# valeoai/PAFUSE

Hardware: AMD Instinct MI355X
Metric: hypotheses/sec through DDIM loop (H3WB 133-kp, P=20, T=10) (higher is better)
Workload: dtype bf16x3 (every fp32 GEMM operand as the exact sum of three bf16 slices, six bf16 MFMA products per fp32-equivalent product, fp32 accumulate; activations, LayerNorm, softmax, attention and everything in memory fp32; the residual stream stored centred on its row means)

## Files before the change

__graft_entry__.py:

```python
import os
import subprocess
import sys

ROOT = os.path.dirname(os.path.abspath(__file__))
if ROOT not in sys.path:
    sys.path.insert(0, ROOT)

SRC = os.path.join(ROOT, "pafuse_amd", "csrc", "pafuse_hip.hip")
CSRC = os.path.join(ROOT, "pafuse_amd", "csrc")
DEPS = [SRC, os.path.join(ROOT, "include", "pafuse_hip.h")] + [os.path.join(CSRC, f) for f in
                                                              ("kernels.hpp", "hgemm.hpp", "xgemm.hpp", "sgemm.hpp", "train_kernels.hpp", "train_host.inc")]
OUT = os.path.join(ROOT, "pafuse_amd", "libpafuse_hip.so")
from pafuse_amd.build_flags import HIPCC_FLAGS

FLAGS_NOTE = OUT + ".flags"


def _stale(out, deps):
    if (not os.path.exists(out)) or any(os.path.getmtime(d) > os.path.getmtime(out) for d in deps):
        return True
    try:
        with open(FLAGS_NOTE) as f:
            return f.read().strip() != " ".join(HIPCC_FLAGS)
    except OSError:
        return True


def hipcc_compile(args, out):
    hipcc = os.environ.get("HIPCC", "/opt/rocm/bin/hipcc")
    cmd = [hipcc] + HIPCC_FLAGS + list(args) + ["-o", out]
    print("[build]", " ".join(cmd), file=sys.stderr, flush=True)
    r = subprocess.run(cmd, stderr=subprocess.PIPE, text=True)
    noise = "is not a recognized feature for this target"
    sys.stderr.write("".join(l for l in r.stderr.splitlines(True) if noise not in l))
# ... 70 lines not shown
```

include/pafuse_hip.h:

```cpp
#ifndef PAFUSE_HIP_H
#define PAFUSE_HIP_H

#include <stddef.h>
#include <stdint.h>

#ifdef __cplusplus
extern "C" {
#endif

#define PAFUSE_OK 0
#define PAFUSE_E_ARG (-1)
#define PAFUSE_E_SHAPE (-2)
#define PAFUSE_E_WORKSPACE (-3)
#define PAFUSE_E_HIP (-4)
#define PAFUSE_E_RANGE (-5)

#define PAFUSE_MAX_DEPTH 16
#define PAFUSE_MAX_PARTS 4

typedef struct pafuse_block_weights {
    const float *norm1_w, *norm1_b;
    const float *qkv_w, *qkv_b;
    const float *proj_w, *proj_b;
    const float *norm2_w, *norm2_b;
// ... 88 lines not shown
    const float *W;
    const void *Wsplit;
    const float *bias;
    const float *resid;
    float *out_x, *out_n;
    const float *post_w, *post_b;
    float post_eps;
    const float *pos;
    int32_t posJ, posF;
    const float *next_w, *next_b;
    float next_eps;
    const float *head_w, *head_b;
    float *out_head;
    float *ln_stats;
    const void *A_img;
    const void *resid_img;
    void *out_x_img, *out_n_img;
    const float *rowscale;
    int32_t rs_temporal, rs_J, rs_FJ;
    float *out_pre;
} pafuse_rowln_args;
int pafuse_linear_rowln(const pafuse_rowln_args *a, void *stream);
int pafuse_linear_rowln_group(const pafuse_rowln_args *a, int32_t n, int32_t shared_grid, void *stream);

int pafuse_layernorm(const float *x, const float *w, const float *b, float *out, int64_t M, int32_t C, float eps,
                     void *stream);

int pafuse_attention(const float *qkv, float *o, int64_t nseq, int32_t L, int32_t C, int32_t heads, int64_t group,
                     int64_t group_stride, int64_t seq_stride, int64_t tok_stride, void *stream);

int pafuse_attention_backward(const float *qkv, const float *d_o, float *dqkv, int64_t nseq, int32_t L, int32_t C, int32_t heads,
                              int64_t group, int64_t group_stride, int64_t seq_stride, int64_t tok_stride, void *stream);
size_t pafuse_linear_weight_grad_bytes(void);
int pafuse_linear_weight_grad(const float *dY, const float *X, float *dW, float *db, int64_t M, int32_t N, int32_t K,
                              int32_t operand_bf16, void *workspace, size_t workspace_bytes, void *stream);

typedef struct pafuse_lnb_args {
    const float *dy, *x, *w;
    float eps;
    const float *add;
    float *dx;
    const float *drop;
    int32_t temporal, J, FJ;
    float *out_scaled;
    float *dw, *db, *dbranch;
    int64_t M;
// ... 214 lines not shown
```

pafuse_amd/_lib.py:

```python
import ctypes as C
import os

_HERE = os.path.dirname(os.path.abspath(__file__))
LIB_PATH = os.path.join(_HERE, "libpafuse_hip.so")

MAX_DEPTH = 16
MAX_PARTS = 4
f32p = C.POINTER(C.c_float)
i32p = C.POINTER(C.c_int32)


BLOCK_FIELDS = ("norm1_w", "norm1_b", "qkv_w", "qkv_b", "proj_w", "proj_b",
                "norm2_w", "norm2_b", "fc1_w", "fc1_b", "fc2_w", "fc2_b")


class BlockWeights(C.Structure):
    _names = ("norm1_w", "norm1_b", "qkv_w", "qkv_b", "proj_w", "proj_b",
              "norm2_w", "norm2_b", "fc1_w", "fc1_b", "fc2_w", "fc2_b",
              "qkv_ws", "proj_ws", "fc1_ws", "fc2_ws",
              "qkv_ls", "qkv_lt", "fc1_ls", "fc1_lt",
              "qkv_hs", "qkv_hb", "qkv_hl", "fc2_hp")
    _fields_ = [(n, C.c_void_p) for n in _names]


# ... 39 lines not shown
                [(n, C.c_int32) for n in ("operand_bf16", "ln_folded", "h_residual_only")] +
                [(n, C.c_void_p) for n in ("x", "xn", "image", "stats")] + [("row0", C.c_int64), ("nrows", C.c_int64)])


class DDIMStep(C.Structure):
    _fields_ = [("time", C.c_int64), ("last", C.c_int32),
                ("sqrt_recip_acp", C.c_double), ("sqrt_recipm1_acp", C.c_double),
                ("sqrt_alpha_next", C.c_double), ("c", C.c_double), ("sigma", C.c_double)]


SIGNATURES = {
    "pafuse_version": (C.c_char_p, []),
    "pafuse_last_error": (C.c_char_p, []),
    "pafuse_abi_version": (C.c_int, []),
    "pafuse_linear": (C.c_int, [C.c_void_p, C.c_void_p, C.c_void_p, C.c_void_p, C.c_int64, C.c_int32, C.c_int32,
                                C.c_int32, C.c_void_p]),
    "pafuse_split_weights_bytes": (C.c_size_t, [C.c_int64, C.c_int64]),
    "pafuse_split_image_bytes": (C.c_size_t, [C.c_int64, C.c_int64, C.c_int32]),
    "pafuse_split_weights": (C.c_int, [C.c_void_p, C.c_int32, C.c_int32, C.c_int32, C.c_void_p, C.c_void_p]),
    "pafuse_linear_split": (C.c_int, [C.c_void_p, C.c_void_p, C.c_void_p, C.c_void_p, C.c_int64, C.c_int32, C.c_int32,
                                      C.c_int32, C.c_void_p]),
    "pafuse_linear_rowln": (C.c_int, [C.POINTER(RowLNArgs), C.c_void_p]),
    "pafuse_linear_rowln_group": (C.c_int, [C.POINTER(RowLNArgs), C.c_int32, C.c_int32, C.c_void_p]),
    "pafuse_hsplit_rows": (C.c_int, [C.c_void_p, C.c_int64, C.c_int32, C.c_void_p, C.c_void_p]),
    "pafuse_xsplit_rows": (C.c_int, [C.c_void_p, C.c_int64, C.c_int32, C.c_void_p, C.c_void_p]),
    "pafuse_linear_x": (C.c_int, [C.c_void_p, C.c_void_p, C.c_void_p, C.c_void_p, C.c_void_p, C.c_int64, C.c_int32, C.c_int32,
                                  C.c_int32, C.c_void_p]),
    "pafuse_linear_h": (C.c_int, [C.c_void_p, C.c_void_p, C.c_void_p, C.c_void_p, C.c_void_p, C.c_int64, C.c_int32, C.c_int32,
                                  C.c_int32, C.c_void_p]),
    "pafuse_qkv_attention_image": (C.c_int, [C.c_int32, C.c_void_p, C.c_void_p, C.c_void_p, C.c_void_p, C.c_void_p, C.c_int64, C.c_int64,
                                             C.c_int32, C.c_int32, C.c_int32, C.c_int64, C.c_int64, C.c_int64, C.c_int64, C.c_float, C.c_void_p]),
    "pafuse_mlp_h": (C.c_int, [C.c_void_p, C.c_void_p, C.c_void_p, C.c_void_p, C.c_void_p, C.c_void_p, C.c_void_p, C.c_void_p,
                               C.c_int64, C.c_int32, C.c_float, C.c_void_p]),
    "pafuse_layernorm": (C.c_int, [C.c_void_p, C.c_void_p, C.c_void_p, C.c_void_p, C.c_int64, C.c_int32, C.c_float,
                                   C.c_void_p]),
    "pafuse_attention": (C.c_int, [C.c_void_p, C.c_void_p, C.c_int64, C.c_int32, C.c_int32, C.c_int32, C.c_int64,
                                   C.c_int64, C.c_int64, C.c_int64, C.c_void_p]),
    "pafuse_attention_backward": (C.c_int, [C.c_void_p, C.c_void_p, C.c_void_p, C.c_int64, C.c_int32, C.c_int32, C.c_int32,
                                            C.c_int64, C.c_int64, C.c_int64, C.c_int64, C.c_void_p]),
    "pafuse_linear_weight_grad_bytes": (C.c_size_t, []),
    "pafuse_linear_weight_grad": (C.c_int, [C.c_void_p, C.c_void_p, C.c_void_p, C.c_void_p, C.c_int64, C.c_int32, C.c_int32,
                                            C.c_int32, C.c_void_p, C.c_size_t, C.c_void_p]),
    "pafuse_train_unit_bytes": (C.c_size_t, [C.c_int64, C.c_int32, C.c_int32]),
    "pafuse_layernorm_backward": (C.c_int, [C.POINTER(LnbArgs), C.c_void_p, C.c_size_t, C.c_void_p]),
    "pafuse_linear_input_grad": (C.c_int, [C.c_void_p, C.c_void_p, C.c_void_p, C.c_void_p, C.c_int64, C.c_int32, C.c_int32,
                                           C.c_int32, C.c_int32, C.c_void_p, C.c_size_t, C.c_void_p]),
# ... 146 lines not shown
```

pafuse_amd/csrc/kernels.hpp:

```cpp
#pragma once
#include <hip/hip_runtime.h>
#include <stdint.h>

#include <utility>

namespace pafuse {

typedef float f32x16 __attribute__((ext_vector_type(16)));
typedef float f32x4 __attribute__((ext_vector_type(4)));

constexpr int BK = 32;
constexpr int LDK = 36;

typedef __bf16 bf16x8 __attribute__((ext_vector_type(8)));
__device__ __forceinline__ bf16x8 to_bf16x8(const f32x4 lo, const f32x4 hi) {
    bf16x8 v;
#pragma unroll
    for (int i = 0; i < 4; ++i) v[i] = (__bf16)lo[i], v[4 + i] = (__bf16)hi[i];
    return v;
}

#ifdef PAFUSE_MFMA_K8
typedef __bf16 bf16x4_t __attribute__((ext_vector_type(4)));
typedef short s16x4_t __attribute__((ext_vector_type(4)));
// ... 234 lines not shown
    v += __shfl_xor(v, 32);
    return half_wave_sum(v);
}

enum { EPI_BIAS = 0, EPI_ROWLN = 1, EPI_ROWLN_TRAIN = 2 };

enum { MODE_F32 = 0, MODE_BF16 = 1, MODE_BF16X3 = 2, MODE_F16X2 = 3, MODE_BF16X3_IMAGES = 4 };
constexpr bool mode_valid(int m) { return m >= MODE_F32 && m <= MODE_BF16X3_IMAGES; }
constexpr bool mode_split(int m) { return m >= MODE_BF16X3; }
constexpr bool mode_images(int m) { return m >= MODE_F16X2; }
constexpr int image_elem_bytes(int m) { return m == MODE_BF16X3_IMAGES ? 6 : 4; }
enum { WLAYOUT_PLAIN = 0, WLAYOUT_ROWLN = 1, WLAYOUT_M16 = 2 };

struct GemmParams {
    const float* A;
    const float* W;
    const float* bias;
    float* out;
    int64_t M;
    int N, K;
    int mode;
    const uint8_t* Wsplit;
    int wlayout;
    int act;
    float* out_act;
    const float* dact_u;
    const float* resid;
    float* out_x;
    float* out_n;
    const float* post_w;
    const float* post_b;
    float post_eps;
    const float* pos;
    int posJ, posF;
    const float* next_w;
    const float* next_b;
    float next_eps;
    const float* head_w;
    const float* head_b;
    float* out_head;
    float* ln_stats;
    const float* ln_in;
    const float* ln_s;
    const uint8_t* Ah;
    const uint8_t* Wh;
    uint8_t* out_h;
// ... 1061 lines not shown
        constexpr auto need = [](int nth) { return (size_t)VEC + 5 * BN + (size_t)NW * 32 * (32 * nth + 4); };
        constexpr int NTH = (NT % 2 == 0 && need(2) <= RINGF) ? 2 : 1;
        static_assert(need(NTH) <= RINGF, "epilogue scratch must fit the ring");
        epilogue_rows_h<WN, NT, BM, NW, NTH, false, 2>(acc, p, m0, n0, wm, wn, r, h, wave, lane, smem, 1.0f);
    } else {
        epilogue_row_per_lane<WN, NT, BM, EPI, VEC>(acc, p, m0, n0, wm, wn, r, h, smem);
    }
}

template <int WM, int WN, int NT, int EPI, int NSTAGE, int MINW, int ABL = 0, int BKC = 32>
__global__ void __launch_bounds__(WM* WN * 64, MINW) gemm_dma_kernel(const GemmParams p) {
    PAFUSE_XQ_GUARD();
    extern __shared__ __attribute__((aligned(16))) float smem[];
    gemm_dma_tile<WM, WN, NT, EPI, NSTAGE, ABL, BKC>(p, blockIdx.x, gridDim.x, smem);
}

constexpr int GROUP_MAX = 4;
struct GroupedGemmParams {
    GemmParams p[GROUP_MAX];
    int first[GROUP_MAX + 1];
    int n;
};

template <int EPI>
__global__ void __launch_bounds__(256, 2) grouped_rowln_kernel(const GroupedGemmParams g) {
    PAFUSE_XQ_GUARD();
    extern __shared__ __attribute__((aligned(16))) float smem[];
    const int b = blockIdx.x;
    int s = 0;
#pragma unroll
    for (int i = 1; i < GROUP_MAX; ++i)
        if (i < g.n && b >= g.first[i]) s = i;
    const GemmParams& p = g.p[s];
    const int lb = b - g.first[s], nb = g.first[s + 1] - g.first[s];
    switch (p.N) {
        case 384: gemm_dma_tile<2, 2, 6, EPI, 2, 0, 16, false>(p, lb, nb, smem); break;
        case 256: gemm_dma_tile<2, 2, 4, EPI, 2, 0, 16, false>(p, lb, nb, smem); break;
        case 224: gemm_dma_tile<4, 1, 7, EPI, 2, 0, 16, false>(p, lb, nb, smem); break;
        default: break;
    }
}

struct AttnParams {
    const float* qkv;
    float* o;
    uint8_t* o_h;
    int64_t nseq;
    int L, C, heads, d;
    int64_t group, group_stride, seq_stride, tok_stride;
    float scale;
};

template <int ITEMS>
__device__ __forceinline__ void attn_item(int64_t i, int64_t nseq, int heads, int64_t& seq, int& head) {
    if (nseq % 8 == 0 && ((nseq / 8) * heads) % ITEMS == 0) {
        const int64_t blk = i / ITEMS;
        const int lo = (int)(blk % 8);
        const int64_t u = (blk / 8) * ITEMS + (i % ITEMS);
        head = (int)(u % heads);
        seq = (u / heads) * 8 + lo;
    } else {
// ... 2565 lines not shown
```

pafuse_amd/csrc/pafuse_hip.hip:

```cpp
#include "../../include/pafuse_hip.h"

#include <hip/hip_runtime.h>

#include <algorithm>
#include <cmath>
#include <cstdarg>
#include <cstdio>
#include <cstdlib>
#include <cstring>
#include <type_traits>

#include "kernels.hpp"
#include "hgemm.hpp"
#include "xgemm.hpp"
#include "sgemm.hpp"
#include "train_kernels.hpp"

using namespace pafuse;

namespace {

thread_local char g_err[512] = "";

int fail(int code, const char* fmt, ...) {
    va_list ap;
    va_start(ap, fmt);
    vsnprintf(g_err, sizeof g_err, fmt, ap);
    va_end(ap);
    return code;
}

int check_launch(const char* what) {
    hipError_t e = hipGetLastError();
    if (e != hipSuccess) return fail(PAFUSE_E_HIP, "%s: %s", what, hipGetErrorString(e));
    return PAFUSE_OK;
}

inline size_t align_up(size_t x, size_t a = 256) { return (x + a - 1) / a * a; }
// ... 231 lines not shown
        case 8: return launch_strip2<NB, 8>(p, s);
        default: return fail(PAFUSE_E_ARG, "strip GEMM: epilogue options %d", flags);
    }
}
int strip2_bias(const GemmParams& p, hipStream_t s) {
    if (p.N % 128 == 0) return launch_strip2_flags<8>(p, s);
    if (p.N % 112 == 0) return launch_strip2_flags<7>(p, s);
    return launch_strip2_flags<6>(p, s);
}

int wsplit_chunk(int N, bool whole_row) { return (whole_row && (N == 384 || N == 288 || N == 256 || N == 224)) ? 16 : 32; }

template <int WM, int WN, int NT, int EPI, int NSTAGE, int MINW, int BKC = 32>
int launch_gemm_dma(const GemmParams& p, hipStream_t s) {
    using T = DmaTile<WM, WN, NT, BKC>;
    constexpr size_t lds = (size_t)NSTAGE * T::STAGE_BYTES;
    static_assert(lds <= 160 * 1024, "LDS budget");
    static_assert(EPI == EPI_BIAS || (size_t)7 * T::BM * WN * sizeof(float) <= lds, "cross-wave reduction scratch must fit");
    if (!p.Wsplit) return fail(PAFUSE_E_ARG, "split-precision GEMM without a pre-split weight image");
    if (p.K % BKC) return fail(PAFUSE_E_SHAPE, "split GEMM: K=%d is not a multiple of %d", p.K, BKC);
    const int64_t tiles = (p.M + T::BM - 1) / T::BM * (p.N / T::BN);
    if (tiles <= 0 || tiles > 0x7fffffff) return fail(PAFUSE_E_ARG, "gemm grid out of range");
    return launch<gemm_dma_kernel<WM, WN, NT, EPI, NSTAGE, MINW, 0, BKC>>("gemm_dma_kernel", (unsigned)tiles, T::NTHR, lds, s, p);
}

template <int WM, int WN, int NT, int EPI, int NSTAGE, int BKC, int MINW, bool HRES = false>
int launch_hgemm(const GemmParams& p, hipStream_t s) {
    using T = HTile<WM, WN, NT, BKC>;
    constexpr size_t lds = (size_t)NSTAGE * T::STAGE_BYTES;
    static_assert(lds <= 160 * 1024, "LDS budget");
    static_assert(EPI == EPI_BIAS || (size_t)7 * T::BM * WN * sizeof(float) <= lds, "cross-wave reduction scratch must fit");
    if (!p.Ah || !p.Wh) return fail(PAFUSE_E_ARG, "f16x2 GEMM without the H images of its operands");
    if (p.K % BKC || p.K <= 0 || p.N % T::BN) return fail(PAFUSE_E_SHAPE, "f16x2 GEMM: N=%d, K=%d do not fit the %d-column tile", p.N, p.K, T::BN);
    if (HRES && !p.resid_h) return fail(PAFUSE_E_ARG, "f16x2 whole-row GEMM: no H-image residual");
    const int64_t tiles = (p.M + T::BM - 1) / T::BM * (p.N / T::BN);
    if (tiles <= 0 || tiles > 0x7fffffff) return fail(PAFUSE_E_ARG, "gemm grid out of range");
    return launch<hgemm_kernel<WM, WN, NT, EPI, NSTAGE, BKC, MINW, HRES>>("hgemm_kernel", (unsigned)tiles, T::NTHR, lds, s, p);
}

bool hgemm_width(int C) { return C == 384 || C == 256 || C == 224; }
bool hgemm_plain_n(int N) { return N > 0 && (N % 128 == 0 || N % 224 == 0); }

int hgemm_bias(const GemmParams& p, hipStream_t s) {
    if (p.M <= 0) return PAFUSE_OK;
    if (p.N % 128 == 0) return launch_hgemm<4, 2, 2, EPI_BIAS, 3, 16, 2>(p, s);
    if (p.N % 224 == 0) return launch_hgemm<4, 1, 7, EPI_BIAS, 3, 16, 2>(p, s);
// ... 118 lines not shown

template <int EPI>
int gemm_rowln_as(const GemmParams& p0, hipStream_t s) {
    GemmParams p = p0;
    if (p.mode == MODE_BF16X3 && (debug_f32_mask() & 2)) p.mode = MODE_F32;
    if (p.M <= 0) return PAFUSE_OK;
    if (p.K % BK || p.K <= 0) return fail(PAFUSE_E_SHAPE, "rowln: K=%d must be a positive multiple of 32", p.K);
    if (p.mode == MODE_F16X2 || p.mode == MODE_BF16X3_IMAGES) {
        if constexpr (EPI == EPI_ROWLN) return p.mode == MODE_F16X2 ? hgemm_rowln(p, s) : xgemm_rowln(p, s);
        else return fail(PAFUSE_E_ARG, "training has no image-pipeline kernels");
    }
    if constexpr (EPI == EPI_ROWLN_TRAIN) {
        if (p.mode == MODE_BF16X3) {
            switch (p.N) {
                case 384: return launch_gemm_dma<2, 2, 6, EPI, 2, 2, 16>(p, s);
                case 256: return launch_gemm_dma<2, 2, 4, EPI, 2, 2, 16>(p, s);
                case 224: if (p.M >= 4096) return launch_gemm_dma<4, 1, 7, EPI, 2, 2, 16>(p, s); break;
                default: break;
            }
            p.mode = MODE_F32;
        }
    }
    if constexpr (EPI == EPI_ROWLN) {
        if (p.mode == MODE_BF16X3) {
            switch (p.N) {
                case 384: return launch_gemm_dma<2, 2, 6, EPI, 2, 2, 16>(p, s);
                case 256: return launch_gemm_dma<2, 2, 4, EPI, 2, 2, 16>(p, s);
                case 288: return launch_gemm_dma<2, 3, 3, EPI, 2, 2, 16>(p, s);
                case 224:
                    return p.M >= 4096 ? launch_gemm_dma<4, 1, 7, EPI, 2, 2, 16>(p, s) : launch_gemm_dma<2, 1, 7, EPI, 2, 2, 16>(p, s);
                case 128: return launch_gemm<1, 4, 1, EPI, 1, 1, 1, 2>(p, s);
                case 64: return launch_gemm<1, 2, 1, EPI, 1, 1, 1, 2>(p, s);
                default: break;
            }
        } else if (p.mode != MODE_F32) {
            switch (p.N) {
                case 384: return launch_gemm<1, 4, 3, EPI, 1, 1, 1, 1>(p, s);
                case 288: return launch_gemm<1, 3, 3, EPI, 1, 1, 1, 1>(p, s);
                case 256: return launch_gemm<2, 2, 4, EPI, 1, 2, 1, 1>(p, s);
                case 224: return launch_gemm<1, 7, 1, EPI, 1, 1, 1, 1>(p, s);
                case 128: return launch_gemm<1, 4, 1, EPI, 1, 1, 1, 1>(p, s);
                case 64: return launch_gemm<1, 2, 1, EPI, 1, 1, 1, 1>(p, s);
                default: break;
            }
        }
    }
    switch (p.N) {
        case 384: return launch_gemm<1, 4, 3, EPI, 1, 1, 1>(p, s);
        case 288: return launch_gemm<1, 3, 3, EPI, 1, 1, 1>(p, s);
        case 256: return launch_gemm<2, 2, 4, EPI, 1, 2, 1>(p, s);
        case 224: return launch_gemm<1, 7, 1, EPI, 1, 1, 1>(p, s);
        case 128: return launch_gemm<1, 4, 1, EPI, 1, 1, 1>(p, s);
        case 64: return launch_gemm<1, 2, 1, EPI, 1, 1, 1>(p, s);
        default: return fail(PAFUSE_E_SHAPE, "no whole-row kernel for channel width %d (have 64,128,224,256,288,384)", p.N);
    }
}

int gemm_rowln(const GemmParams& p, hipStream_t s) { return gemm_rowln_as<EPI_ROWLN>(p, s); }
int gemm_rowln_train(const GemmParams& p, hipStream_t s) { return gemm_rowln_as<EPI_ROWLN_TRAIN>(p, s); }

bool group_ok_rowln(const GemmParams& p) {
    return p.mode == MODE_BF16X3 && p.Wsplit && (p.N == 384 || p.N == 256 || (p.N == 224 && p.M >= 4096)) && p.K % 16 == 0 && p.K > 0 &&
           !(debug_f32_mask() & 2);
}

template <bool ROWLN>
int gemm_group(const GemmParams* ps, int n, hipStream_t s, bool shared_grids) {
    bool ok = ROWLN && shared_grids && n >= 2 && n <= GROUP_MAX;
    for (int i = 0; i < n && ok; ++i) ok = ps[i].M > 0 && group_ok_rowln(ps[i]);
    if (!ok) {
        for (int i = 0; i < n; ++i) {
            const int rc = ROWLN ? gemm_rowln(ps[i], s) : gemm_bias(ps[i], s);
            if (rc) return rc;
        }
        return PAFUSE_OK;
    }
    int order[GROUP_MAX];
    double cost[GROUP_MAX];
    int64_t tiles[GROUP_MAX];
    for (int i = 0; i < n; ++i) {
        const GemmParams& p = ps[i];
        int bm, bn;
        bm = p.N == 224 ? 128 : 64, bn = p.N;
        tiles[i] = (p.M + bm - 1) / bm * (p.N / bn);
        cost[i] = (double)bm * bn * p.K;
        order[i] = i;
    }
    std::sort(order, order + n, [&](int a, int b) { return cost[a] > cost[b]; });
    GroupedGemmParams g{};
    g.n = n;
    int64_t first = 0;
    for (int k = 0; k < n; ++k) {
        g.p[k] = ps[order[k]];
        g.first[k] = (int)first;
        first += (tiles[order[k]] + 7) / 8 * 8;
        if (first > 0x7fffffff) return fail(PAFUSE_E_ARG, "grouped gemm grid out of range");
    }
    g.first[n] = (int)first;
    for (int k = n + 1; k <= GROUP_MAX; ++k) g.first[k] = (int)first;
    constexpr size_t lds = 2 * DmaTile<2, 2, 6, 16>::STAGE_BYTES;
    static_assert(lds >= 2 * DmaTile<2, 2, 4, 16>::STAGE_BYTES && lds >= 2 * DmaTile<4, 1, 7, 16>::STAGE_BYTES && lds <= 80 * 1024, "LDS");
    return launch<grouped_rowln_kernel<EPI_ROWLN>>("grouped_rowln_kernel", (unsigned)first, 256, lds, s, g);
}

bool width_supported(int C) { return C == 384 || C == 288 || C == 256 || C == 224 || C == 128 || C == 64; }

template <int LP, int DP, int NW>
int launch_attn(const AttnParams& p, hipStream_t s) {
    constexpr int ITEMS = NW / (LP / 16);
    constexpr size_t lds = (size_t)2 * ITEMS * LP * (DP + 4) * sizeof(float);
    const int64_t nitems = p.nseq * p.heads;
    const int64_t grid = (nitems + ITEMS - 1) / ITEMS;
    if (grid > 0x7fffffff) return fail(PAFUSE_E_ARG, "attention grid out of range");
    return launch<attn_kernel<LP, DP, NW>>("attn_kernel", (unsigned)grid, NW * 64, lds, s, p);
}

template <int DP>
int launch_attn_long(const AttnParams& p, hipStream_t s) {
    constexpr size_t lds = (size_t)2 * ATTN_LONG_LP * (DP + 4) * sizeof(float);
    static_assert(lds <= 160 * 1024, "LDS");
    const int64_t grid = p.nseq * p.heads;
    if (grid > 0x7fffffff) return fail(PAFUSE_E_ARG, "attention grid out of range");
    return launch<attn_long_kernel<DP>>("attn_long_kernel", (unsigned)grid, 1024, lds, s, p);
}

// ... 534 lines not shown
    g.A = a->A, g.W = a->W, g.bias = a->bias, g.M = a->M, g.N = a->N, g.K = a->K, g.mode = mode;
    g.Wsplit = mode == MODE_BF16X3 ? (const uint8_t*)a->Wsplit : nullptr;
    g.resid = a->resid, g.out_x = a->out_x, g.out_n = a->out_n;
    g.post_w = a->post_w, g.post_b = a->post_b, g.post_eps = a->post_eps;
    g.pos = a->pos, g.posJ = a->posJ, g.posF = a->posF;
    g.next_w = a->next_w, g.next_b = a->next_b, g.next_eps = a->next_eps;
    g.head_w = a->head_w, g.head_b = a->head_b, g.out_head = a->out_head;
    g.ln_stats = a->ln_stats;
    if (img) {
        g.Ah = (const uint8_t*)a->A_img, g.Wh = (const uint8_t*)a->Wsplit;
        g.resid_h = (const uint8_t*)a->resid_img;
        g.out_xh = (uint8_t*)a->out_x_img, g.out_nh = (uint8_t*)a->out_n_img;
    }
    g.rowscale = a->rowscale, g.rs_temporal = a->rs_temporal, g.rs_J = a->rs_J, g.rs_FJ = a->rs_FJ, g.out_pre = a->out_pre;
    return PAFUSE_OK;
}

int pafuse_linear_rowln(const pafuse_rowln_args* a, void* stream) {
    StreamDevice on_stream_device(stream);
    GemmParams g;
    const int rc = rowln_params(a, g);
    if (rc) return rc;
    if (g.M == 0) return PAFUSE_OK;
    return a->training ? gemm_rowln_train(g, (hipStream_t)stream) : gemm_rowln(g, (hipStream_t)stream);
}

int pafuse_linear_rowln_group(const pafuse_rowln_args* a, int32_t n, int32_t shared_grid, void* stream) {
    StreamDevice on_stream_device(stream);
    if (!a || n < 1 || n > GROUP_MAX) return fail(PAFUSE_E_ARG, "linear_rowln_group: %d layers (1 .. %d)", n, GROUP_MAX);
    GemmParams g[GROUP_MAX];
    int live = 0;
    for (int i = 0; i < n; ++i) {
        const int rc = rowln_params(&a[i], g[live]);
        if (rc) return rc;
        if (a[i].training) return fail(PAFUSE_E_ARG, "linear_rowln_group: training layers run one by one (pafuse_linear_rowln)");
        if (g[live].M > 0) ++live;
    }
    if (!live) return PAFUSE_OK;
    return gemm_group<true>(g, live, (hipStream_t)stream, shared_grid != 0);
}

int pafuse_hsplit_rows(const float* X, int64_t R, int32_t K, void* out, void* stream) {
    StreamDevice on_stream_device(stream);
    if (!X || !out || R < 0) return fail(PAFUSE_E_ARG, "hsplit_rows: null pointer or negative row count");
    if (K <= 0 || K % 8) return fail(PAFUSE_E_SHAPE, "hsplit_rows: K=%d must be a positive multiple of 8", K);
    if (R == 0) return PAFUSE_OK;
// ... 1415 lines not shown
```

pafuse_amd/ops.py:

```python
import ctypes as C
import math
from operator import attrgetter

import torch

from . import _lib
from ._lib import IMAGE_BYTES, MODE_BF16X3, MODE_F16X2, PRECISIONS, SPLIT_FLAG
from .images import _ptr, block_images, effective_mode, fill_block_struct, fused_mlp_fc2_image, head_major_qkv, split_image


def _stream(t):
    return torch.cuda.current_stream(t.device).cuda_stream


def _need(cond, msg):
    if not cond:
        raise ValueError(msg)


def _data(t):
    return t.data_ptr() if t.numel() else None


def _need_pred(who, pred, axis="P_r"):
# ... 623 lines not shown
        a.rs_temporal, a.rs_J, a.rs_FJ = (int(v) for v in rs_map)
        a.out_pre = buf("pre", (M, N))
    keep += [post, pos, next, head, rowscale]

    def finish():
        join = hjoin_rows if mode == MODE_F16X2 else xjoin_rows
        res = {}
        for name in ("x", "n", "pre"):
            if name in out and out[name] is not None and (name != "x" or not resid_image):
                res[name] = out[name].reshape(-1)[:M * N].view(M, N)
        for name, cols in (("head", 3), ("stats", 2)):
            if name in out:
                res[name] = out[name].reshape(-1)[:M * cols].view(M, cols)
        for name in ("x_img", "n_img"):
            if name in out:
                res[name] = join(out[name].reshape(-1)[:M * N * eb], M, N)
        if resid_image:
            res["x"] = res["x_img"]
        return res

    return a, keep, finish


def linear_rowln(x, weight, bias, resid, precision="bf16x3", **options):
    lib = _lib.load()
    a, keep, finish = rowln_args(x, weight, bias, resid, precision, **options)
    with torch.cuda.device(x.device):
        _lib.check(lib.pafuse_linear_rowln(C.byref(a), _stream(x)))
    del keep
    return finish()


def linear_rowln_group(layers, shared_grid=True):
    lib = _lib.load()
    _need(1 <= len(layers) <= _lib.MAX_PARTS, f"linear_rowln_group: 1 .. {_lib.MAX_PARTS} layers")
    built = [rowln_args(**layer) for layer in layers]
    arr = (_lib.RowLNArgs * len(built))(*[b[0] for b in built])
    dev = layers[0]["x"].device
    with torch.cuda.device(dev):
        _lib.check(lib.pafuse_linear_rowln_group(arr, len(built), int(bool(shared_grid)), _stream(layers[0]["x"])))
    return [b[2]() for b in built]


def procrustes_errors(pred, gt, x2d, traj, cam, conn, pick=True):
    lib = _lib.load()
    _need(pred.dim() == 6 and pred.shape[-1] == 3, f"procrustes_errors: pred must be [B,T,P,F,J,3], got {tuple(pred.shape)}")
    B, T, P, F, J, _ = pred.shape
    _need(tuple(gt.shape) == (B, F, J, 3) and tuple(x2d.shape) == (B, F, J, 2) and traj.numel() == B * F * 3
          and cam.numel() == 9 and conn.numel() == J, "procrustes_errors: operands do not match pred")
    _need_tensors("procrustes_errors", (pred, gt, x2d, traj, cam), (conn,))
    dev = pred.device
# ... 665 lines not shown
```

Before: 106.0.

## Add full-row strip GEMM tile for bf16x3 row-LayerNorm epilogue layers

Adds a new kernel tile for the GEMM+row-LayerNorm epilogue in which each workgroup computes a 64-row strip across the full output width (224/256/384). It streams pre-split weight slabs through double-buffered LDS via global_load_lds, interleaves the bf16x3 splitting of the next A chunk with the MFMAs, and does the LN and head epilogue directly from registers. This path becomes the default for single and grouped rowln launches in bf16x3 mode. The aim is to remove cross-tile reduction and LDS traffic for row statistics and improve weight streaming. The cost is higher register pressure and a tightly hand-scheduled pipeline, and the grouped path now requires K to be a multiple of 32.

Measured after the change: 106.9, median of 6. Within noise of the previous version (+0.8%).

```diff
diff --git a/__graft_entry__.py b/__graft_entry__.py
--- a/__graft_entry__.py
+++ b/__graft_entry__.py
@@ -9,7 +9,7 @@
 SRC = os.path.join(ROOT, "pafuse_amd", "csrc", "pafuse_hip.hip")
 CSRC = os.path.join(ROOT, "pafuse_amd", "csrc")
 DEPS = [SRC, os.path.join(ROOT, "include", "pafuse_hip.h")] + [os.path.join(CSRC, f) for f in
-                                                              ("kernels.hpp", "hgemm.hpp", "xgemm.hpp", "sgemm.hpp", "train_kernels.hpp", "train_host.inc")]
+                                                              ("kernels.hpp", "hgemm.hpp", "xgemm.hpp", "sgemm.hpp", "rowln_strip.hpp", "train_kernels.hpp", "train_host.inc")]
 OUT = os.path.join(ROOT, "pafuse_amd", "libpafuse_hip.so")
 from pafuse_amd.build_flags import HIPCC_FLAGS
 
diff --git a/include/pafuse_hip.h b/include/pafuse_hip.h
--- a/include/pafuse_hip.h
+++ b/include/pafuse_hip.h
@@ -134,6 +134,7 @@
 } pafuse_rowln_args;
 int pafuse_linear_rowln(const pafuse_rowln_args *a, void *stream);
 int pafuse_linear_rowln_group(const pafuse_rowln_args *a, int32_t n, int32_t shared_grid, void *stream);
+int pafuse_linear_rowln_tile(const pafuse_rowln_args *a, int32_t tile, void *stream);
 
 int pafuse_layernorm(const float *x, const float *w, const float *b, float *out, int64_t M, int32_t C, float eps,
                      void *stream);
diff --git a/pafuse_amd/_lib.py b/pafuse_amd/_lib.py
--- a/pafuse_amd/_lib.py
+++ b/pafuse_amd/_lib.py
@@ -85,6 +85,7 @@
                                       C.c_int32, C.c_void_p]),
     "pafuse_linear_rowln": (C.c_int, [C.POINTER(RowLNArgs), C.c_void_p]),
     "pafuse_linear_rowln_group": (C.c_int, [C.POINTER(RowLNArgs), C.c_int32, C.c_int32, C.c_void_p]),
+    "pafuse_linear_rowln_tile": (C.c_int, [C.POINTER(RowLNArgs), C.c_int32, C.c_void_p]),
     "pafuse_hsplit_rows": (C.c_int, [C.c_void_p, C.c_int64, C.c_int32, C.c_void_p, C.c_void_p]),
     "pafuse_xsplit_rows": (C.c_int, [C.c_void_p, C.c_int64, C.c_int32, C.c_void_p, C.c_void_p]),
     "pafuse_linear_x": (C.c_int, [C.c_void_p, C.c_void_p, C.c_void_p, C.c_void_p, C.c_void_p, C.c_int64, C.c_int32, C.c_int32,
diff --git a/pafuse_amd/csrc/kernels.hpp b/pafuse_amd/csrc/kernels.hpp
--- a/pafuse_amd/csrc/kernels.hpp
+++ b/pafuse_amd/csrc/kernels.hpp
@@ -280,6 +280,7 @@
     int mode;
     const uint8_t* Wsplit;
     int wlayout;
+    int rowln_tile;
     int act;
     float* out_act;
     const float* dact_u;
@@ -1387,7 +1388,12 @@
     int n;
 };
 
-template <int EPI>
+template <int NB, int UB>
+__device__ __forceinline__ void rowln_strip_tile(const GemmParams& p, const int b, const int nb, float* smem);
+enum { ROWLN_STRIP_384 = 1, ROWLN_STRIP_256 = 2, ROWLN_STRIP_224 = 4 };
+constexpr int rowln_strip_bit(int N) { return N == 384 ? ROWLN_STRIP_384 : N == 256 ? ROWLN_STRIP_256 : N == 224 ? ROWLN_STRIP_224 : 0; }
+
+template <int EPI, int STRIP = 0>
 __global__ void __launch_bounds__(256, 2) grouped_rowln_kernel(const GroupedGemmParams g) {
     PAFUSE_XQ_GUARD();
     extern __shared__ __attribute__((aligned(16))) float smem[];
@@ -1399,9 +1405,18 @@
     const GemmParams& p = g.p[s];
     const int lb = b - g.first[s], nb = g.first[s + 1] - g.first[s];
     switch (p.N) {
-        case 384: gemm_dma_tile<2, 2, 6, EPI, 2, 0, 16, false>(p, lb, nb, smem); break;
-        case 256: gemm_dma_tile<2, 2, 4, EPI, 2, 0, 16, false>(p, lb, nb, smem); break;
-        case 224: gemm_dma_tile<4, 1, 7, EPI, 2, 0, 16, false>(p, lb, nb, smem); break;
+        case 384:
+            if constexpr (STRIP & ROWLN_STRIP_384) rowln_strip_tile<24, 8>(p, lb, nb, smem);
+            else gemm_dma_tile<2, 2, 6, EPI, 2, 0, 16, false>(p, lb, nb, smem);
+            break;
+        case 256:
+            if constexpr (STRIP & ROWLN_STRIP_256) rowln_strip_tile<16, 8>(p, lb, nb, smem);
+            else gemm_dma_tile<2, 2, 4, EPI, 2, 0, 16, false>(p, lb, nb, smem);
+            break;
+        case 224:
+            if constexpr (STRIP & ROWLN_STRIP_224) rowln_strip_tile<14, 7>(p, lb, nb, smem);
+            else gemm_dma_tile<4, 1, 7, EPI, 2, 0, 16, false>(p, lb, nb, smem);
+            break;
         default: break;
     }
 }
diff --git a/pafuse_amd/csrc/pafuse_hip.hip b/pafuse_amd/csrc/pafuse_hip.hip
--- a/pafuse_amd/csrc/pafuse_hip.hip
+++ b/pafuse_amd/csrc/pafuse_hip.hip
@@ -14,6 +14,7 @@
 #include "hgemm.hpp"
 #include "xgemm.hpp"
 #include "sgemm.hpp"
+#include "rowln_strip.hpp"
 #include "train_kernels.hpp"
 
 using namespace pafuse;
@@ -291,6 +292,30 @@
     const int64_t tiles = (p.M + T::BM - 1) / T::BM * (p.N / T::BN);
     if (tiles <= 0 || tiles > 0x7fffffff) return fail(PAFUSE_E_ARG, "gemm grid out of range");
     return launch<gemm_dma_kernel<WM, WN, NT, EPI, NSTAGE, MINW, 0, BKC>>("gemm_dma_kernel", (unsigned)tiles, T::NTHR, lds, s, p);
+}
+
+#ifndef PAFUSE_ROWLN_STRIP
+#define PAFUSE_ROWLN_STRIP (ROWLN_STRIP_384 | ROWLN_STRIP_256 | ROWLN_STRIP_224)
+#endif
+bool rowln_strip_on(const GemmParams& p) {
+    const int bit = rowln_strip_bit(p.N);
+    if (!bit || p.mode != MODE_BF16X3) return false;
+    return p.rowln_tile ? p.rowln_tile == 2 : (PAFUSE_ROWLN_STRIP & bit) != 0;
+}
+template <int NB, int UB>
+int launch_rowln_strip(const GemmParams& p, hipStream_t s) {
+    using T = RowStripTile<NB, UB>;
+    if (!p.Wsplit) return fail(PAFUSE_E_ARG, "split-precision GEMM without a pre-split weight image");
+    const int64_t tiles = (p.M + T::BM - 1) / T::BM;
+    if (tiles <= 0 || tiles > 0x7fffffff) return fail(PAFUSE_E_ARG, "gemm grid out of range");
+    return launch<rowln_strip_kernel<NB, UB>>("rowln_strip_kernel", (unsigned)tiles, T::NTHR, T::LDS_BYTES, s, p);
+}
+int rowln_strip(const GemmParams& p, hipStream_t s) {
+    switch (p.N) {
+        case 384: return launch_rowln_strip<24, 8>(p, s);
+        case 256: return launch_rowln_strip<16, 8>(p, s);
+        default: return launch_rowln_strip<14, 7>(p, s);
+    }
 }
 
 template <int WM, int WN, int NT, int EPI, int NSTAGE, int BKC, int MINW, bool HRES = false>
@@ -455,6 +480,9 @@
         }
     }
     if constexpr (EPI == EPI_ROWLN) {
+        if (p.rowln_tile && (p.mode != MODE_BF16X3 || !rowln_strip_bit(p.N)))
+            return fail(PAFUSE_E_SHAPE, "rowln: a named tile needs mode 2 and a width of 224, 256 or 384 (mode %d, width %d)", p.mode, p.N);
+        if (rowln_strip_on(p)) return rowln_strip(p, s);
         if (p.mode == MODE_BF16X3) {
             switch (p.N) {
                 case 384: return launch_gemm_dma<2, 2, 6, EPI, 2, 2, 16>(p, s);
@@ -493,8 +521,8 @@
 int gemm_rowln_train(const GemmParams& p, hipStream_t s) { return gemm_rowln_as<EPI_ROWLN_TRAIN>(p, s); }
 
 bool group_ok_rowln(const GemmParams& p) {
-    return p.mode == MODE_BF16X3 && p.Wsplit && (p.N == 384 || p.N == 256 || (p.N == 224 && p.M >= 4096)) && p.K % 16 == 0 && p.K > 0 &&
-           !(debug_f32_mask() & 2);
+    return p.mode == MODE_BF16X3 && p.Wsplit && (p.N == 384 || p.N == 256 || (p.N == 224 && (p.M >= 4096 || rowln_strip_on(p)))) && p.K % 32 == 0 && p.K > 0 &&
+           !p.rowln_tile && !(debug_f32_mask() & 2);
 }
 
 template <bool ROWLN>
@@ -514,7 +542,7 @@
     for (int i = 0; i < n; ++i) {
         const GemmParams& p = ps[i];
         int bm, bn;
-        bm = p.N == 224 ? 128 : 64, bn = p.N;
+        bm = (p.N == 224 && !rowln_strip_on(p)) ? 128 : 64, bn = p.N;
         tiles[i] = (p.M + bm - 1) / bm * (p.N / bn);
         cost[i] = (double)bm * bn * p.K;
         order[i] = i;
@@ -533,7 +561,8 @@
     for (int k = n + 1; k <= GROUP_MAX; ++k) g.first[k] = (int)first;
     constexpr size_t lds = 2 * DmaTile<2, 2, 6, 16>::STAGE_BYTES;
     static_assert(lds >= 2 * DmaTile<2, 2, 4, 16>::STAGE_BYTES && lds >= 2 * DmaTile<4, 1, 7, 16>::STAGE_BYTES && lds <= 80 * 1024, "LDS");
-    return launch<grouped_rowln_kernel<EPI_ROWLN>>("grouped_rowln_kernel", (unsigned)first, 256, lds, s, g);
+    static_assert(lds >= RowStripTile<24, 8>::LDS_BYTES && lds >= RowStripTile<16, 8>::LDS_BYTES && lds >= RowStripTile<14, 7>::LDS_BYTES, "LDS");
+    return launch<grouped_rowln_kernel<EPI_ROWLN, PAFUSE_ROWLN_STRIP>>("grouped_rowln_kernel", (unsigned)first, 256, lds, s, g);
 }
 
 bool width_supported(int C) { return C == 384 || C == 288 || C == 256 || C == 224 || C == 128 || C == 64; }
@@ -1114,6 +1143,18 @@
     const int rc = rowln_params(a, g);
     if (rc) return rc;
     if (g.M == 0) return PAFUSE_OK;
+    return a->training ? gemm_rowln_train(g, (hipStream_t)stream) : gemm_rowln(g, (hipStream_t)stream);
+}
+
+int pafuse_linear_rowln_tile(const pafuse_rowln_args* a, int32_t tile, void* stream) {
+    StreamDevice on_stream_device(stream);
+    if (tile < 0 || tile > 2) return fail(PAFUSE_E_ARG, "linear_rowln_tile: tile %d (0 the dispatch's, 1 LDS-DMA, 2 strip)", tile);
+    GemmParams g;
+    const int rc = rowln_params(a, g);
+    if (rc) return rc;
+    if (tile && a->training) return fail(PAFUSE_E_ARG, "linear_rowln_tile: training layers have one tile (pafuse_linear_rowln)");
+    if (g.M == 0) return PAFUSE_OK;
+    g.rowln_tile = tile;
     return a->training ? gemm_rowln_train(g, (hipStream_t)stream) : gemm_rowln(g, (hipStream_t)stream);
 }
 
diff --git a/pafuse_amd/csrc/rowln_strip.hpp b/pafuse_amd/csrc/rowln_strip.hpp
--- /dev/null
+++ b/pafuse_amd/csrc/rowln_strip.hpp
@@ -0,0 +1,298 @@
+#pragma once
+#include "sgemm.hpp"
+
+namespace pafuse {
+
+template <int NB, int UB>
+struct RowStripTile {
+    static_assert(NB % UB == 0, "whole column units");
+    static constexpr int NW = 4, NTHR = 256, BM = 64, BN = NB * 16;
+    static constexpr int CT = NB / UB;
+    static constexpr int SLAB_BYTES = UB * 16 * 96;
+    static constexpr int UNIT_BYTES = 2 * SLAB_BYTES;
+    static constexpr int A_WAVE = 2048, A_STAGE = NW * A_WAVE;
+    static constexpr int A_BASE = 2 * UNIT_BYTES;
+    static constexpr int IA = 2;
+    static constexpr int IWT = UNIT_BYTES / 1024, IW = (IWT + NW - 1) / NW;
+    static constexpr size_t LDS_BYTES = (size_t)A_BASE + 2 * A_STAGE;
+    static_assert(UNIT_BYTES % 1024 == 0, "whole DMA pieces");
+    static_assert(LDS_BYTES <= 80 * 1024, "two workgroups per CU");
+};
+
+template <int NB, int UB>
+__device__ __forceinline__ void rowln_strip_tile(const GemmParams& p, const int b, const int nb, float* smem) {
+    using T = RowStripTile<NB, UB>;
+    constexpr int CT = T::CT, IW = T::IW, IWT = T::IWT, IA = T::IA;
+    constexpr int TOT = UB * 6;
+    constexpr int NSPLIT = 4 * 5;
+    static_assert(TOT >= 36 && 4 * (IW - 1) + 1 <= TOT / 2, "filler schedule needs room: every W' piece of a unit in front of its A pieces");
+    uint8_t* const lds = reinterpret_cast<uint8_t*>(smem);
+    const uint32_t lds0 = (uint32_t)(size_t)(__attribute__((address_space(3))) void*)smem;
+    const int tid = threadIdx.x, lane = tid & 63;
+    const int wave = __builtin_amdgcn_readfirstlane(tid >> 6);
+    const int c = lane & 15, qd = lane >> 4;
+    int tile;
+    {
+        const int xcd = b & 7, q = nb >> 3, rem = nb & 7;
+        tile = (xcd < rem ? xcd * (q + 1) : rem * (q + 1) + (xcd - rem) * q) + (b >> 3);
+    }
+    const int64_t m0 = (int64_t)tile * T::BM;
+    if (m0 >= p.M) return;
+    const int K = p.K, nk = K / 32;
+
+    const float* a_src[IA];
+#pragma unroll
+    for (int j = 0; j < IA; ++j) {
+        const int64_t row = m0 + wave * 16 + 8 * j + (lane >> 3);
+        const int x = (4 * (j & 1) + (lane >> 4)) & 7;
+        const int ch = (lane & 7) ^ strip_f(x);
+        a_src[j] = p.A + (row < p.M ? row : p.M - 1) * K + 4 * ch;
+    }
+    const int64_t slab_stride = (int64_t)p.N * 96;
+    int w_off[IW];
+#pragma unroll
+    for (int j = 0; j < IW; ++j) {
+        int i = wave + j * T::NW;
+        i = i < IWT ? i : IWT - 1;
+        const int s16 = i * 64 + lane, row = s16 / 12, q = s16 % 12;
+        const int sb = ((q / 3) - (row >> 1)) & 3;
+        w_off[j] = (sb >> 1) * (int)slab_stride + row * 96 + (((sb & 1) + (row >> 3)) & 1) * 48 + (q % 3) * 16;
+    }
+    auto issue_w = [&](int j, int g, int ct, int slot) {
+        int i = wave + j * T::NW;
+        i = i < IWT ? i : IWT - 1;
+        const uint8_t* const src = p.Wsplit + 2 * g * slab_stride + ct * T::SLAB_BYTES + w_off[j];
+        __builtin_amdgcn_global_load_lds((const __attribute__((address_space(1))) void*)src,
+                                         (__attribute__((address_space(3))) void*)(lds + slot * T::UNIT_BYTES + i * 1024), 16, 0, 0);
+    };
+    auto issue_a = [&](int j, int kc) {
+        const int k = kc < nk ? kc : nk - 1;
+        __builtin_amdgcn_global_load_lds((const __attribute__((address_space(1))) void*)(a_src[j] + k * 32),
+                                         (__attribute__((address_space(3))) void*)(lds + T::A_BASE + (kc & 1) * T::A_STAGE + wave * T::A_WAVE + j * 1024),
+                                         16, 0, 0);
+    };
+
+    const int fc = strip_f((c >> 1) & 7);
+    const uint32_t a_frag = (uint32_t)(T::A_BASE + wave * T::A_WAVE + c * 128 + (((2 * qd) ^ fc) * 16));
+    const uint32_t w_frag = (uint32_t)(c * WSPLIT_ROW_BYTES + wsplit_sub_offset<32, 1>(c, qd));
+
+    f32x4 acc[NB];
+#pragma unroll
+    for (int n = 0; n < NB; ++n) acc[n] = f32x4{0.f, 0.f, 0.f, 0.f};
+    u32x4 cur[3];
+    SplitPair sp[4];
+
+#pragma unroll
+    for (int s = 0; s < 2; ++s)
+#pragma unroll
+        for (int j = 0; j < IA; ++j) issue_a(j, s);
+#pragma unroll
+    for (int j = 0; j < IW; ++j) issue_w(j, 0, 0, 0);
+    wait_vmcnt<0>();
+    {
+        u32x4 lo = lds_read128<0>(lds0 + a_frag), hi = lds_read128<0>(lds0 + (a_frag ^ 16u));
+        asm volatile("s_waitcnt lgkmcnt(0)" : "+v"(lo), "+v"(hi));
+        const bf16x8x3 s3 = split3(__builtin_bit_cast(f32x4, lo), __builtin_bit_cast(f32x4, hi));
+        cur[0] = __builtin_bit_cast(u32x4, s3.s0), cur[1] = __builtin_bit_cast(u32x4, s3.s1), cur[2] = __builtin_bit_cast(u32x4, s3.s2);
+    }
+    asm volatile("" ::: "memory");
+#pragma unroll
+    for (int j = 0; j < IA; ++j) issue_a(j, 2);
+
+    for (int g = 0; g < nk; ++g) {
+        static_for<CT>([&](auto CT_) {
+            constexpr int ct = decltype(CT_)::value;
+            const int u = g * CT + ct;
+            wait_vmcnt<ct == 1 ? IA : 0>();
+            __builtin_amdgcn_s_barrier();
+            const uint32_t sbase = lds0 + (uint32_t)((u & 1) * T::UNIT_BYTES);
+            constexpr int nct = (ct + 1) % CT;
+            const int ng = ct + 1 < CT ? g : (g + 1 < nk ? g + 1 : g);
+
+            __builtin_amdgcn_s_setprio(1);
+            u32x4 n_lo, n_hi;
+            if constexpr (ct == 0) {
+                const uint32_t anext = lds0 + (uint32_t)(((g + 1) & 1) * T::A_STAGE);
+                n_lo = lds_read128<0>(anext + a_frag);
+                n_hi = lds_read128<0>(anext + (a_frag ^ 16u));
+            }
+            u32x4 wf[2][3];
+            auto load_w = [&](auto N_) {
+                constexpr int n = decltype(N_)::value;
+                constexpr int off = n * 16 * WSPLIT_ROW_BYTES;
+                const uint32_t addr = sbase + w_frag;
+                wf[n & 1][0] = lds_read128<off>(addr);
+                wf[n & 1][1] = lds_read128<off + 16>(addr);
+                wf[n & 1][2] = lds_read128<off + 32>(addr);
+            };
+            load_w(std::integral_constant<int, 0>{});
+
+            static_for<UB>([&](auto N_) {
+                constexpr int n = decltype(N_)::value;
+                if constexpr (n + 1 < UB) {
+                    load_w(std::integral_constant<int, n + 1>{});
+                    if constexpr (n == 0 && ct == 0) {
+                        asm volatile("s_waitcnt lgkmcnt(3)" : "+v"(n_lo), "+v"(n_hi), "+v"(wf[0][0]), "+v"(wf[0][1]), "+v"(wf[0][2]));
+#pragma unroll
+                        for (int q = 0; q < 4; ++q) {
+                            sp[q].x0 = __builtin_bit_cast(float, q < 2 ? n_lo[2 * q] : n_hi[2 * q - 4]);
+                            sp[q].x1 = __builtin_bit_cast(float, q < 2 ? n_lo[2 * q + 1] : n_hi[2 * q - 3]);
+                        }
+                    } else {
+                        asm volatile("s_waitcnt lgkmcnt(3)" : "+v"(wf[n & 1][0]), "+v"(wf[n & 1][1]), "+v"(wf[n & 1][2]));
+                    }
+                } else {
+                    asm volatile("s_waitcnt lgkmcnt(0)" : "+v"(wf[n & 1][0]), "+v"(wf[n & 1][1]), "+v"(wf[n & 1][2]));
+                }
+                const u32x4(&w)[3] = wf[n & 1];
+                static_for<6>([&](auto S_) {
+                    constexpr int pi = decltype(S_)::value;
+                    constexpr int t = n * 6 + pi;
+                    constexpr int wi = pi == 0 ? 0 : pi == 1 ? 2 : pi == 2 ? 1 : pi == 3 ? 0 : pi == 4 ? 1 : 0;
+                    constexpr int ai = pi == 0 ? 2 : pi == 1 ? 0 : pi == 2 ? 1 : pi == 3 ? 1 : pi == 4 ? 0 : 0;
+                    constexpr int na = ct * UB + n;
+                    SGEMM_PIN_ACC(acc[na]);
+                    acc[na] = mfma16_bf16_k32(__builtin_bit_cast(bf16x8, w[wi]), __builtin_bit_cast(bf16x8, cur[ai]), acc[na]);
+                    if constexpr (t % 4 == 1 && t / 4 < IW) {
+                        asm volatile("" ::: "memory");
+                        issue_w(t / 4, ng, nct, (u + 1) & 1);
+                        asm volatile("" ::: "memory");
+                    }
+                    if constexpr (ct == 0) {
+                        constexpr int T0 = 6, SPAN = TOT - T0 - 2;
+                        if constexpr (t >= T0) {
+                            constexpr int k_lo = ((t - T0) * NSPLIT + SPAN - 1) / SPAN;
+                            constexpr int k_hi = ((t - T0 + 1) * NSPLIT + SPAN - 1) / SPAN;
+                            static_for<(k_hi < NSPLIT ? k_hi : NSPLIT) - (k_lo < NSPLIT ? k_lo : NSPLIT)>([&](auto K_) {
+                                constexpr int k = k_lo + decltype(K_)::value;
+                                constexpr int stage = k / 4, sq = k % 4;
+                                SGEMM_PIN_PAIR(sp[sq]);
+                                sp[sq].template stage<stage>();
+                                SGEMM_PIN_PAIR(sp[sq]);
+                            });
+                        }
+                        if constexpr (t >= TOT / 2 && t < TOT / 2 + 3 * IA && (t - TOT / 2) % 3 == 0) {
+                            asm volatile("" ::: "memory");
+                            issue_a((t - TOT / 2) / 3, g + 3);
+                            asm volatile("" ::: "memory");
+                        }
+                    }
+                });
+            });
+            __builtin_amdgcn_s_setprio(0);
+        });
+#pragma unroll
+        for (int q = 0; q < 4; ++q) cur[0][q] = sp[q].s0, cur[1][q] = sp[q].s1, cur[2][q] = sp[q].s2;
+    }
+    wait_vmcnt<0>();
+
+    const int64_t m = m0 + wave * 16 + c;
+    const bool live = m < p.M;
+    const int64_t mm = live ? m : p.M - 1;
+    const int N = p.N;
+    const float invC = 1.0f / (float)N;
+    auto row_sum = [&](float v) {
+        v += __shfl_xor(v, 16);
+        v += __shfl_xor(v, 32);
+        return v;
+    };
+    auto vec4 = [&](const float* v, int n) { return *reinterpret_cast<const f32x4*>(v + 16 * n + 4 * qd); };
+    auto lane_sum = [&](const float (&s4)[4]) { return (s4[0] + s4[1]) + (s4[2] + s4[3]); };
+    auto stats = [&](float eps, float& mean, float& rstd) {
+        float s4[4] = {0.f, 0.f, 0.f, 0.f};
+#pragma unroll
+        for (int n = 0; n < NB; ++n)
+#pragma unroll
+            for (int e = 0; e < 4; ++e) s4[e] += acc[n][e];
+        mean = row_sum(lane_sum(s4)) * invC;
+        asm volatile("" : "+v"(mean));
+        float q4[4] = {0.f, 0.f, 0.f, 0.f};
+#pragma unroll
+        for (int n = 0; n < NB; ++n)
+#pragma unroll
+            for (int e = 0; e < 4; ++e) {
+                const float d = acc[n][e] - mean;
+                q4[e] = fmaf(d, d, q4[e]);
+            }
+        rstd = 1.0f / sqrtf(fmaf(row_sum(lane_sum(q4)), invC, eps));
+    };
+    auto layer_norm = [&](float eps, const float* gw, const float* gb) {
+        float mean, rstd;
+        stats(eps, mean, rstd);
+#pragma unroll
+        for (int n = 0; n < NB; ++n) {
+            const f32x4 g4 = vec4(gw, n), b4 = vec4(gb, n);
+#pragma unroll
+            for (int e = 0; e < 4; ++e) acc[n][e] = fmaf((acc[n][e] - mean) * rstd, g4[e], b4[e]);
+        }
+    };
+    auto store_rows = [&](float* dst) {
+        if (live) {
+            float* const row = dst + m * N + 4 * qd;
+#pragma unroll
+            for (int n = 0; n < NB; ++n) *reinterpret_cast<f32x4*>(row + 16 * n) = acc[n];
+        }
+    };
+    {
+        const float* const rrow = p.resid + mm * N;
+#pragma unroll
+        for (int n = 0; n < NB; ++n) {
+            const f32x4 b4 = vec4(p.bias, n), r4 = vec4(rrow, n);
+#pragma unroll
+            for (int e = 0; e < 4; ++e) acc[n][e] = (acc[n][e] + b4[e]) + r4[e];
+        }
+    }
+    if (p.post_w) layer_norm(p.post_eps, p.post_w, p.post_b);
+    if (p.pos) {
+        const float* const pe = p.pos + (int64_t)((mm / p.posJ) % p.posF) * N;
+#pragma unroll
+        for (int n = 0; n < NB; ++n) {
+            const f32x4 e4 = vec4(pe, n);
+#pragma unroll
+            for (int e = 0; e < 4; ++e) acc[n][e] += e4[e];
+        }
+    }
+    if (p.next_w && p.ln_stats) {
+        float mean, rstd;
+        stats(p.next_eps, mean, rstd);
+        if (live && qd == 0) {
+            p.ln_stats[2 * m] = mean;
+            p.ln_stats[2 * m + 1] = rstd;
+        }
+        if (p.out_x) {
+#pragma unroll
+            for (int n = 0; n < NB; ++n)
+#pragma unroll
+                for (int e = 0; e < 4; ++e) acc[n][e] -= mean;
+            store_rows(p.out_x);
+        }
+        return;
+    }
+    if (p.out_x) store_rows(p.out_x);
+    if (!p.next_w) return;
+    layer_norm(p.next_eps, p.next_w, p.next_b);
+    if (p.out_n) store_rows(p.out_n);
+    if (p.out_head) {
+#pragma unroll
+        for (int k = 0; k < 3; ++k) {
+            float s4[4] = {0.f, 0.f, 0.f, 0.f};
+#pragma unroll
+            for (int n = 0; n < NB; ++n) {
+                const f32x4 hw = vec4(p.head_w + k * N, n);
+#pragma unroll
+                for (int e = 0; e < 4; ++e) s4[e] = fmaf(acc[n][e], hw[e], s4[e]);
+            }
+            const float s = row_sum(lane_sum(s4));
+            if (live && qd == 0) p.out_head[m * 3 + k] = s + p.head_b[k];
+        }
+    }
+}
+
+template <int NB, int UB>
+__global__ void __launch_bounds__(256, 2) rowln_strip_kernel(const GemmParams p) {
+    PAFUSE_XQ_GUARD();
+    extern __shared__ __attribute__((aligned(16))) float smem[];
+    rowln_strip_tile<NB, UB>(p, blockIdx.x, gridDim.x, smem);
+}
+
+}
diff --git a/pafuse_amd/ops.py b/pafuse_amd/ops.py
--- a/pafuse_amd/ops.py
+++ b/pafuse_amd/ops.py
@@ -669,11 +669,18 @@
     return a, keep, finish
 
 
-def linear_rowln(x, weight, bias, resid, precision="bf16x3", **options):
-    lib = _lib.load()
+ROWLN_TILES = {None: 0, "dma": 1, "strip": 2}
+
+
+def linear_rowln(x, weight, bias, resid, precision="bf16x3", tile=None, **options):
+    lib = _lib.load()
+    _need(tile in ROWLN_TILES, f"linear_rowln: tile must be one of {list(ROWLN_TILES)}")
     a, keep, finish = rowln_args(x, weight, bias, resid, precision, **options)
     with torch.cuda.device(x.device):
-        _lib.check(lib.pafuse_linear_rowln(C.byref(a), _stream(x)))
+        if tile is None:
+            _lib.check(lib.pafuse_linear_rowln(C.byref(a), _stream(x)))
+        else:
+            _lib.check(lib.pafuse_linear_rowln_tile(C.byref(a), ROWLN_TILES[tile], _stream(x)))
     del keep
     return finish()
 
```
